# SKIRT/SKIRT9

Measured on AMD Instinct MI355X. Metric: photon packets/s (whole node), 10^6-cell octree, higher is better.
Workload: dtype f64

## Files before the change

### skirt9_amd/csrc/pmc_context.h

```cpp
#ifndef PMC_CONTEXT_H
#define PMC_CONTEXT_H

#include "pmc_device.h"
#include "../../include/pmc_layout.h"
#include "../../include/pmc_tuning.h"
#include <hip/hip_runtime.h>
#include <algorithm>
#include <chrono>
#include <cmath>
#include <cstdio>
#include <rccl/rccl.h>
#include <cstdlib>
#include <cstring>
#include <deque>
#include <atomic>
#include <mutex>
#include <string>
#include <thread>
#include <map>
#include <vector>

extern "C" const char* pmcTune(const char* name);
extern "C" hipError_t pmcUploadScene(int slot, const DevScene* scene, hipStream_t stream);
extern "C" hipError_t pmcConfigureKernels(size_t walkLds, size_t transitionLds);
extern "C" int pmcWalkBlocksPerCU(int gridKind, int kind, int wide, int block, size_t ldsBytes);
extern "C" hipError_t pmcLaunchStatMerge(int slot, int blocks, hipStream_t stream);
extern "C" int pmcPeelBlock(void);
extern "C" int pmcPropBlock(void);
extern "C" hipError_t pmcLaunchWalk(int slot, int gridKind, int flavour, int taskBase, int numTaskRecords, int taskCounter, uint64_t seed, int grid,
                                    int block, size_t ldsBytes, const WalkStreamArgs* tasks, hipStream_t stream);
extern "C" hipError_t pmcLaunchPeel(int slot, int form, int slotBase, int numSlots, const int* list, int cursor, int obs, int sgn, int grid, size_t ldsBytes,
                                    const PeelRec* sortedRec, const unsigned long long* sortedCount, unsigned long long* xcdCursor, hipStream_t stream);
extern "C" int pmcVoroPropWavesPerSimd(void);
extern "C" hipError_t pmcLaunchVoroProp(int slot, const int32_t* list, const unsigned long long* count, unsigned long long* xcdCursor, int segments, uint64_t seed,
                                        int flavour, int grid, hipStream_t stream);
extern "C" int pmcVoroPeelWavesPerSimd(void);
extern "C" hipError_t pmcLaunchVoroPeel(int slot, int rec, int tab, const int32_t* list, const unsigned long long* count, unsigned long long* xcdCursor, int segments,
                                        int severalMedia, int grid, hipStream_t stream);
extern "C" hipError_t pmcLaunchProp(int slot, int wide, int flavour, int checkpoints, int slotBase, int numSlots, const int* list, int cursor, uint64_t seed,
                                    int grid, size_t ldsBytes, const RfLogArgs* rfLog, hipStream_t stream);
extern "C" hipError_t pmcLaunchRfFlush(int slot, const uint32_t* keys, const double* vals, uint32_t* sortedKeys, double* sortedVals, unsigned long long n,
                                       int numParts, void* temp, int numCU, hipStream_t stream);
extern "C" int pmcPeelHasQueues(int form, size_t ldsBytes);
extern "C" int pmcPropHasCheckpoints(int flavour, size_t ldsBytes);
extern "C" int pmcExperimentBuild(void);
extern "C" const unsigned long long* pmcPeelSortedCount(void* temp);
extern "C" size_t pmcPeelSortTempBytes();
extern "C" hipError_t pmcLaunchPeelSortCounts(int slot, int slotBase, int numSlots, PeelSortArgs* ps, PeelRec* const* sorted, int32_t* const* lists, void* const* temp,
                                              int* groups, hipStream_t stream);
extern "C" size_t pmcRfTempBytes(int numParts);
extern "C" int pmcRfMaxParts();
extern "C" hipError_t pmcLaunchDipoleCosines(const double* u, int64_t n, double* out, hipStream_t stream);
extern "C" hipError_t pmcLaunchTransition(int slot, int dipole, int slotBase, int numSlots, int group, uint64_t seed, const int* list, int listLen, int maxBlocks,
                                          size_t ldsBytes, const StatLogArgs* statLog, uint64_t count, hipStream_t stream);
extern "C" hipError_t pmcLaunchLaunch(int slot, int slotBase, int numSlots, int group, uint64_t first, uint64_t count, uint64_t seed, int initial,
                                      int maxBlocks, size_t ldsBytes, const StatLogArgs* statLog, hipStream_t stream);
extern "C" hipError_t pmcLaunchStatFlush(int slot, const uint32_t* keys, const double* vals, uint32_t* sortedKeys, double* sortedVals, unsigned long long n,
                                         int numParts, void* temp, int numCU, const uint32_t* chunkFill, hipStream_t stream);
extern "C" int pmcStatBucketBits();
extern "C" hipError_t pmcLaunchCycleStart(int slot, int gridKind, int slotBase, int numSlots, int listCounter, int* listOut, const int* listIn,
                                          int listLen, int maxBlocks, size_t ldsBytes, const PeelSortArgs* sort, hipStream_t stream);
extern "C" hipError_t pmcLaunchTrace(int slot, int gridKind, int wide, int uniform, const double r[3], const double k[3],
                                     const double* kdev, int32_t* m, double* ds, int32_t cap, int32_t* n, size_t ldsBytes,
                                     hipStream_t stream);

void pmcSetError(const std::string& message);
namespace
{
    inline int fail(int code, const std::string& message)
    {
        pmcSetError(message);
        return code;
    }
    inline int hipFail(hipError_t e, const char* what)
    {
        return fail(PMC_ERR_DEVICE, std::string(what) + ": " + hipGetErrorString(e));
    }
}

#define HIP_TRY(call)                                           \
    do                                                          \
    {                                                           \
// ... 132 lines not shown
```

### skirt9_amd/csrc/pmc_device.h

```cpp
#ifndef PMC_DEVICE_H
#define PMC_DEVICE_H

#include "../../include/pmc.h"
#include <stdint.h>

#define PMC_MAX_INSTRUMENTS 16
#define PMC_MAX_CONTEXTS 6
#define PMC_MAX_LEVEL 20
#define PMC_STAT_CAP 48
#define PMC_STAT_POOL_EXHAUSTED 0x40000000

#define PMC_LINK_NONE 0x7FFFFFFFu
#define PMC_LINK_NODE 0x80000000u
#define PMC_LINK_OCTET 0x40000000u
#define PMC_LINK_EXP_BITS 5
#define PMC_LINK_EXP_MASK 31u
#define PMC_LINK_INDEX_MASK 0x1FFFFFFu
#define PMC_LINK_MAX_INDEX ((1u << 25) - 2u)

struct CellRec
{
    double   density;
    uint32_t link[6];
};
// ... 232 lines not shown
    int cursor;
    unsigned long long* waveBase;
    uint32_t* waveFill;
    uint32_t* chunkFill;
};
#define PMC_STAT_NO_CHUNK 0xFFFFFFFFu
#define PMC_STAT_LOG_WAVES 16384
#define PMC_STAT_BUCKET_BITS 11

struct PeelRec
{
    double rx, ry, rz;
    double ds;
    double target;
    uint64_t pidx;
    uint32_t cell, bits;
    int32_t slot;
    uint32_t pad;
};
#define PMC_SORT_OBS 4
struct PeelSortArgs
{
    int32_t numObs;
    int32_t propIndex;
    int32_t obs[PMC_SORT_OBS];
    int8_t sortIndex[16];
    PeelRec* out[PMC_SORT_OBS];
    int32_t* listOut[PMC_SORT_OBS];
    uint32_t* matrix[PMC_SORT_OBS];
    const unsigned long long* start[PMC_SORT_OBS];
    uint32_t numParts;
    uint32_t cap;
    int32_t ldsOffset;
    double centre[3];
    double scale;
};
struct WalkStreamArgs
{
    int32_t numLists;
    int32_t rec[PMC_SORT_OBS];
    const int32_t* list[PMC_SORT_OBS];
    const unsigned long long* count[PMC_SORT_OBS];
    unsigned long long* xcdCursor;
    const int32_t* propList;
    const unsigned long long* propCount;
};
struct PeelSortedArgs
{
    const PeelRec* rec;
    const unsigned long long* count;
    unsigned long long* xcdCursor;
};
#ifndef PMC_PEEL_TILES
#define PMC_PEEL_TILES 32
#endif
#define PMC_VORO_RUN_UNIT_BITS 27
#define PMC_VORO_RUN_UNIT_MASK 0x07FFFFFFu
#define PMC_VORO_RUN_COUNT_UNKNOWN 31u
#define PMC_VORO_FIRST_SCAN (-1000)
#define PMC_VORO_RUN_PAD 16
#ifndef PMC_VORO_RUN_LANES
#define PMC_VORO_RUN_LANES 2
#endif
#ifndef PMC_VORO_CONES
#define PMC_VORO_CONES 192
#endif
// ... 20 lines not shown
```

### skirt9_amd/csrc/pmc_kernels.hip

```cpp

#include "pmc_device.h"
#include "../../include/pmc_philox.h"
#include <hip/hip_runtime.h>
#include <cstdlib>
#include <cstring>
#include <float.h>
#include <math.h>
#include <algorithm>
#include <mutex>
#include <array>
#include <type_traits>
#include <utility>

#ifndef PMC_WALK_REFILL
    #define PMC_WALK_REFILL 40
#endif
#ifndef PMC_PEEL_REFILL
    #define PMC_PEEL_REFILL 32
#endif
#ifndef PMC_PROP_REFILL
    #define PMC_PROP_REFILL 40
#endif
#ifndef PMC_PEEL_BLOCK
    #define PMC_PEEL_BLOCK 768
// ... 314 lines not shown
{
    WalkStreamArgs ws;
    std::memset(&ws, 0, sizeof(ws));
    if (tasks) ws = *tasks;
    const WalkKernel kernel = walkKernels[(flavour & 7) | (gridKind == PMC_GRID_VORONOI ? 8 : 0)].kernel;
    hipLaunchKernelGGL(kernel, dim3(grid), dim3(block), ldsBytes, stream, slot, taskBase, numTaskRecords, taskCounter, seed, ws);
    return hipGetLastError();
}

extern "C" int pmcVoroPeelWavesPerSimd(void) { return PMC_VPEEL_MIN_WAVES; }
extern "C" hipError_t pmcLaunchVoroPeel(int slot, int rec, int tab, const int32_t* list, const unsigned long long* count, unsigned long long* xcdCursor, int segments,
                                        int severalMedia, int grid, hipStream_t stream)
{
    hipLaunchKernelGGL(severalMedia ? voroPeelKernel<true> : voroPeelKernel<false>, dim3(grid), dim3(256), 0, stream, slot, rec, tab, list, count, xcdCursor,
                       segments);
    return hipGetLastError();
}

extern "C" int pmcVoroPropWavesPerSimd(void) { return PMC_VPROP_MIN_WAVES; }
extern "C" hipError_t pmcLaunchVoroProp(int slot, const int32_t* list, const unsigned long long* count, unsigned long long* xcdCursor, int segments, uint64_t seed,
                                        int flavour, int grid, hipStream_t stream)
{
    hipLaunchKernelGGL(voroPropKernels[flavour & 7], dim3(grid), dim3(256), 0, stream, slot, list, count, xcdCursor, segments, seed);
    return hipGetLastError();
}

constexpr int PEEL_SORT_GROUPS = 1024;
constexpr int PEEL_SORT_PARTS = PMC_PEEL_TILES * PMC_PEEL_TILES;
extern "C" size_t pmcPeelSortTempBytes()
{
    return (size_t(2) * PEEL_SORT_PARTS + 2) * sizeof(unsigned long long) + size_t(PEEL_SORT_GROUPS) * PEEL_SORT_PARTS * sizeof(uint32_t);
}
extern "C" const unsigned long long* pmcPeelSortedCount(void* temp) { return static_cast<const unsigned long long*>(temp) + 2 * PEEL_SORT_PARTS; }
extern "C" hipError_t pmcLaunchPeelSortCounts(int slot, int slotBase, int numSlots, PeelSortArgs* ps, PeelRec* const* sorted, int32_t* const* lists, void* const* temp,
                                              int* groups, hipStream_t stream)
{
    ps->numParts = PEEL_SORT_PARTS;
    const int numLists = ps->numObs + (ps->propIndex >= 0 ? 1 : 0);
    for (int k = 0; k < numLists; ++k)
    {
        unsigned long long* totals = static_cast<unsigned long long*>(temp[k]);
        ps->out[k] = sorted ? sorted[k] : nullptr;
        ps->listOut[k] = lists ? lists[k] : nullptr;
        ps->matrix[k] = reinterpret_cast<uint32_t*>(totals + 2 * PEEL_SORT_PARTS + 2);
        ps->start[k] = totals + PEEL_SORT_PARTS;
    }
    const int tiles = (numSlots + PEEL_SORT_TILE - 1) / PEEL_SORT_TILE;
    *groups = std::max(1, std::min(tiles, PEEL_SORT_GROUPS));
    hipLaunchKernelGGL(peelSortCountKernel, dim3(*groups), dim3(256), 0, stream, slot, slotBase, numSlots, *ps);
    for (int k = 0; k < numLists; ++k)
    {
        unsigned long long* totals = static_cast<unsigned long long*>(temp[k]);
        hipLaunchKernelGGL(peelSortOffsetsKernel, dim3((PEEL_SORT_PARTS + 15) / 16), dim3(256), 0, stream, ps->matrix[k], (uint32_t)*groups, (uint32_t)PEEL_SORT_PARTS, totals);
        hipLaunchKernelGGL(rfScanKernel, dim3(1), dim3(PMC_SCAN_THREADS), 0, stream, totals, totals + PEEL_SORT_PARTS, (uint32_t)PEEL_SORT_PARTS);
    }
    return hipGetLastError();
}

extern "C" hipError_t pmcLaunchPeel(int slot, int form, int slotBase, int numSlots, const int* list, int cursor, int obs, int sgn, int grid, size_t ldsBytes,
                                    const PeelRec* sortedRec, const unsigned long long* sortedCount, unsigned long long* xcdCursor, hipStream_t stream)
{
    if (!(form & 4))
        hipLaunchKernelGGL(peelKernels[form & 3].kernel, dim3(grid), dim3(PMC_PEEL_BLOCK), ldsBytes, stream, slot, slotBase, numSlots, cursor, obs, list);
    else
    {
        const size_t queueOffset = (ldsBytes + 15) & ~size_t(15);
        const PeelSortedArgs sorted = {sortedRec, sortedCount, xcdCursor};
        hipLaunchKernelGGL(peel2Kernels[(form & 1) * 8 + (sgn & 7)].kernel, dim3(grid), dim3(PMC_PEEL_BLOCK), queueOffset + pmcPeelQueueBytes(), stream, slot,
                           slotBase, numSlots, cursor, obs, (int)queueOffset, list, sorted);
    }
    return hipGetLastError();
}

extern "C" hipError_t pmcLaunchProp(int slot, int wide, int flavour, int checkpoints, int slotBase, int numSlots, const int* list, int cursor, uint64_t seed,
                                    int grid, size_t ldsBytes, const RfLogArgs* rfLog, hipStream_t stream)
{
    const PropKernel kernel = propKernels[(flavour & 7) | (wide ? 8 : 0)].kernel;
    const size_t trimOffset = (ldsBytes + 15) & ~size_t(15);
    RfLogArgs none = {nullptr, nullptr, 0ull, 0, 0u};
    hipLaunchKernelGGL(kernel, dim3(grid), dim3(PMC_PROP_BLOCK), checkpoints ? trimOffset + PROP_CKPT_BYTES : ldsBytes, stream, slot, slotBase, numSlots, cursor,
                       seed, checkpoints ? (int)trimOffset : -1, rfLog ? *rfLog : none, list);
    return hipGetLastError();
// ... 122 lines not shown
```

### skirt9_amd/csrc/pmc_run.hip

```cpp
#include "pmc_context.h"

namespace
{
    int allocateSlotArrays(pmc_ctx* ctx, int64_t n);
    void releaseSlots(pmc_ctx* ctx)
    {
        for (void* p : ctx->slotAllocations) hipFree(p);
        ctx->slotAllocations.clear();
        ctx->allocatedSlots = 0;
    }

    int allocateSlots(pmc_ctx* ctx, int64_t n)
    {
        hipSetDevice(ctx->device);
        releaseSlots(ctx);
        ctx->planning = true;
        ctx->plannedBytes = 0;
        int rc = allocateSlotArrays(ctx, n);
        ctx->planning = false;
        if (rc) return rc;
        size_t freeBytes = 0, totalBytes = 0;
        if (!ctx->slotsConfigured && n > (int64_t(1) << 20) && hipMemGetInfo(&freeBytes, &totalBytes) == hipSuccess && ctx->plannedBytes > freeBytes / 2)
        {
            const int64_t less = std::max<int64_t>(int64_t(1) << 20, n / 2);
// ... 81 lines not shown
                if (hipMemcpy(ctx->statPoolIota, iota.data(), iota.size() * sizeof(int32_t), hipMemcpyHostToDevice) != hipSuccess)
                    return fail(PMC_ERR_DEVICE, "hipMemcpy failed");
                ctx->statPoolBlocks = blocks;
            }
        }
        TaskArrays& K = ctx->dev.tasks;
        std::memset(&K, 0, sizeof(K));
        const size_t nt = size_t(n) * size_t(1 + ctx->dev.num_instruments);
        double** tdbl[] = {&K.rx, &K.ry, &K.rz, &K.kx, &K.ky, &K.kz, &K.s0, &K.ds, &K.target};
        for (double** d : tdbl)
            if ((rc = ctx->allocate<double>(nt, d, false, &own))) return rc;
        int32_t** tints[] = {&K.cell, &K.cijk};
        for (int32_t** d : tints)
            if ((rc = ctx->allocate<int32_t>(nt, d, false, &own))) return rc;
        if ((rc = ctx->allocate<uint32_t>(size_t(n) / 64 + 64, &K.endedCount, true, &own))) return rc;
        if ((rc = ctx->allocate<int32_t>(2 * size_t(n), &K.liveList, false, &own))) return rc;
        if ((rc = ctx->allocate<uint32_t>(nt, &K.bits, false, &own))) return rc;
    if (ctx->dev.grid_kind == PMC_GRID_OCTREE && (rc = ctx->allocate<uint64_t>(nt, &K.pidx, false, &own))) return rc;
        if (ctx->planning) return PMC_OK;
        A.num_slots = n;
        ctx->allocatedSlots = n;
        ctx->sceneDirty = true;
        return PMC_OK;
    }
}

int pmcAllocateSlots(pmc_ctx* ctx, int64_t n)
{
    return allocateSlots(ctx, n);
}

namespace
{
    struct SegmentPlan
    {
        uint64_t first, count, seed;
        int G;
        int base[PMC_MAX_GROUPS], size[PMC_MAX_GROUPS];
        bool octree;
        int walkFlavour;
        int peelForm;
        bool propCheckpoints;
        int numSortObs, sortObs[PMC_SORT_OBS];
        int propSortIndex, numSortLists;
        PeelSortArgs sortArgs;
        bool sparseLists;
        int listTasksPerLane;
        bool rfLogged, statLogged;
        int rfBuckets, statParts;
        uint32_t rfPadKey;
        unsigned long long rfLogPerSlot, statLogEntries;
        bool poolGrows;
        int statInstruments;
        int launchBlocks, cycleBlocks, transitionBlocks;
        int voroPropGrid, voroPeelGrid, voroPropSegments;
        bool serialWalks, genDump, xcdAffinity, voroPeelKernels, voroPropKernel, voroWalksInSeries;
    };
    struct SegmentRun
    {
        bool active[PMC_MAX_GROUPS], haveWalk[PMC_MAX_GROUPS];
        bool listBuilt[PMC_MAX_GROUPS];
        int listHalf[PMC_MAX_GROUPS];
        bool peelSorted[PMC_MAX_GROUPS];
        bool poolCannotGrow;
        float walkMs, transMs, peelMs, propMs;
        int generations;
    };

    int provisionSlots(pmc_ctx* ctx, uint64_t count, int* numSlots)
    {
        const int64_t want = std::min<int64_t>(ctx->numSlots, (int64_t)std::min<uint64_t>(count, uint64_t(1) << 30));
        bool grow = want > ctx->allocatedSlots;
        if (grow && ctx->allocatedSlots > 0 && ctx->steppedDownFree)
        {
            size_t freeBytes = 0, totalBytes = 0;
            grow = hipMemGetInfo(&freeBytes, &totalBytes) == hipSuccess && freeBytes > ctx->steppedDownFree + ctx->steppedDownFree / 4;
        }
        if (grow)
        {
            HIP_TRY(hipStreamSynchronize(ctx->stream));
            ctx->steppedDownFree = 0;
            int rc = allocateSlots(ctx, want);
            if (rc) return rc;
        }
        *numSlots = (int)std::min<int64_t>(want, ctx->allocatedSlots);
        if (ctx->sceneDirty)
        {
            HIP_TRY(hipStreamSynchronize(ctx->stream));
            HIP_TRY(pmcUploadScene(ctx->slot, &ctx->dev, ctx->stream));
            ctx->sceneDirty = false;
        }
        return PMC_OK;
    }

    SegmentPlan planSegment(const pmc_ctx* ctx, int numSlots, uint64_t first, uint64_t count, uint64_t seed)
    {
        const DevScene& D = ctx->dev;
        SegmentPlan P;
        std::memset(&P, 0, sizeof(P));
        P.first = first, P.count = count, P.seed = seed;
        P.octree = D.grid_kind == PMC_GRID_OCTREE;
        P.serialWalks = pmcTune("PMC_SERIAL_WALKS") != nullptr;
        P.genDump = pmcTune("PMC_GEN_DUMP") != nullptr;
        const bool peelSort = pmcTune("PMC_NO_PEEL_SORT") == nullptr;
        int G = ctx->numGroups;
        if (numSlots < G * 65536) G = 1;
        {
            int observers = 0;
            for (int i = 0; i < D.num_instruments; ++i) observers += D.inst[i].same_observer ? 0 : 1;
            if (D.grid_kind == PMC_GRID_VORONOI && observers <= PMC_SORT_OBS && !ctx->groupsConfigured && peelSort) G = 1;
        }
        P.G = G;
        const int per = ((numSlots + G - 1) / G + PMC_TRANSITION_ALIGN - 1) / PMC_TRANSITION_ALIGN * PMC_TRANSITION_ALIGN;
        for (int g = 0; g < G; ++g)
        {
            P.base[g] = std::min(numSlots, g * per);
            P.size[g] = std::min(per, numSlots - P.base[g]);
        }
        P.walkFlavour = (D.rf_store ? 1 : 0) | (D.explicit_absorption ? 2 : 0) | (D.num_media > 1 ? 4 : 0);
        P.peelForm = (ctx->wide ? 1 : 0) | (D.num_media > 1 ? 2 : 0);
        if (pmcPeelHasQueues(P.peelForm, ctx->walkLds)) P.peelForm |= 4;
        P.propCheckpoints = pmcPropHasCheckpoints(P.walkFlavour, ctx->walkLds);
        P.propSortIndex = -1;
        if (peelSort && (!P.octree || (P.peelForm & 4)))
        {
            int observers = 0;
            for (int i = 0; i < D.num_instruments; ++i)
                if (!D.inst[i].same_observer)
                {
                    if (observers < PMC_SORT_OBS) P.sortObs[observers] = i;
                    ++observers;
                }
            if (observers <= PMC_SORT_OBS) P.numSortObs = observers;
        }
        if (!P.octree && P.numSortObs > 0 && P.numSortObs < PMC_SORT_OBS && pmcTune("PMC_NO_PROP_SORT") == nullptr) P.propSortIndex = P.numSortObs;
        P.numSortLists = P.numSortObs + (P.propSortIndex >= 0 ? 1 : 0);
        PeelSortArgs& sa = P.sortArgs;
        sa.numObs = P.numSortObs;
        sa.propIndex = P.propSortIndex;
        for (int i = 0; i < 16; ++i) sa.sortIndex[i] = -1;
        for (int k = 0; k < P.numSortObs; ++k) sa.obs[k] = P.sortObs[k], sa.sortIndex[P.sortObs[k]] = (int8_t)k;
        const double gdx = D.gx1 - D.gx0, gdy = D.gy1 - D.gy0, gdz = D.gz1 - D.gz0;
        sa.centre[0] = 0.5 * (D.gx0 + D.gx1), sa.centre[1] = 0.5 * (D.gy0 + D.gy1), sa.centre[2] = 0.5 * (D.gz0 + D.gz1);
        sa.scale = PMC_PEEL_TILES / std::sqrt(gdx * gdx + gdy * gdy + gdz * gdz);
        P.xcdAffinity = pmcTune("PMC_NO_XCD_AFFINITY") == nullptr;
        P.sparseLists = P.octree && pmcTune("PMC_NO_LIVE_LISTS") == nullptr;
        P.listTasksPerLane = 1;
        if (const char* env = pmcTune("PMC_LIST_TASKS_PER_LANE")) P.listTasksPerLane = std::max(1, atoi(env));
        P.voroPeelKernels = D.grid_kind == PMC_GRID_VORONOI && pmcTune("PMC_VORO_NO_PEEL_KERNEL") == nullptr;
        P.voroPropKernel = D.grid_kind == PMC_GRID_VORONOI && D.vgen_run && pmcTune("PMC_VORO_NO_PROP_KERNEL") == nullptr
                           && !(pmcTune("PMC_VORO_PLAIN_PROP_ONLY") && (D.num_media > 1 || D.rf_store || D.explicit_absorption));
        P.voroWalksInSeries = pmcTune("PMC_VORO_WALKS_IN_SERIES") != nullptr;
        P.voroPropSegments = (P.xcdAffinity && pmcTune("PMC_VPROP_XCD_SEGMENTS")) ? 8 : 1;
        int propBlocks = pmcVoroPropWavesPerSimd(), peelBlocks = pmcVoroPeelWavesPerSimd();
        if (const char* v = pmcTune("PMC_VPROP_BLOCKS_PER_CU")) propBlocks = std::max(1, atoi(v));
        if (const char* v = pmcTune("PMC_VPEEL_BLOCKS_PER_CU")) peelBlocks = std::max(1, atoi(v));
        P.voroPropGrid = ctx->numCU * propBlocks, P.voroPeelGrid = ctx->numCU * peelBlocks;
        const int64_t rfKeys = P.octree ? int64_t(D.cell_slots) * D.rf_num_lambda : ctx->rfSize;
        const int64_t rfParts = (rfKeys + (int64_t(1) << PMC_RF_BUCKET_BITS) - 1) >> PMC_RF_BUCKET_BITS;
        P.rfLogged = D.rf_store && P.octree && rfParts <= pmcRfMaxParts() && pmcTune("PMC_RF_ATOMICS") == nullptr;
        if (D.rf_store && P.octree && rfParts > pmcRfMaxParts())
        {
            static std::atomic<bool> said{false};
            if (!said.exchange(true))
                fprintf(stderr, "libpmc: the radiation field table has %lld entries, more than the log's counting sort partitions (%d x %d): contributions are added atomically\n",
                        (long long)rfKeys, pmcRfMaxParts(), 1 << PMC_RF_BUCKET_BITS);
        }
        P.rfBuckets = P.rfLogged ? int(rfParts) : 0;
        P.rfPadKey = uint32_t(P.rfBuckets) << PMC_RF_BUCKET_BITS;
        P.rfLogPerSlot = 128ull;
        if (const char* env = pmcTune("PMC_RF_LOG_PER_SLOT")) P.rfLogPerSlot = std::max(1, atoi(env));
        const int statBits = pmcStatBucketBits();
        P.statParts = int((D.stat_acc_records + (int64_t(1) << statBits) - 1) >> statBits);
        P.statLogged = D.any_stats && D.stat_acc_records > 0 && P.statParts <= pmcRfMaxParts() && pmcTune("PMC_STAT_ATOMICS") == nullptr;
        unsigned long long entries = (128ull << 20);
        if (const char* env = pmcTune("PMC_STAT_LOG_ENTRIES")) entries = std::max(1, atoi(env));
        P.statLogEntries = std::max<unsigned long long>((entries + PMC_RF_LOG_CHUNK - 1) / PMC_RF_LOG_CHUNK, 1ull) * PMC_RF_LOG_CHUNK;
        for (int i = 0; i < D.num_instruments; ++i) P.statInstruments += D.inst[i].record_stats ? 1 : 0;
        P.poolGrows = D.any_stats && ctx->statPoolBlocks > 0 && pmcTune("PMC_STAT_POOL_NO_GROWTH") == nullptr;
// ... 219 lines not shown
            D.stat_pool_first[h] = first;
            D.stat_pool_count[h] = count;
            first += count;
        }
        freeNow[g] += (unsigned long long)add;
        HIP_TRY(hipMemcpy(ctr + PMC_CTR_STATFREE(0), freeNow, sizeof(freeNow), hipMemcpyHostToDevice));
        ctx->release(D.stat_pool_bin, own), ctx->release(D.stat_pool_w, own), ctx->release(D.stat_pool_next, own), ctx->release(D.stat_pool_free, own);
        ctx->release(ctx->statPoolIota, own);
        D.stat_pool_bin = bin, D.stat_pool_w = w, D.stat_pool_next = next, D.stat_pool_free = stack;
        ctx->statPoolIota = iota;
        ctx->statPoolBlocks = old + add;
        ctx->readback[g].statFreeBlocks = freeNow[g];
        ctx->statPoolGrowths += 1;
        HIP_TRY(pmcUploadScene(ctx->slot, &D, ctx->stream));
        HIP_TRY(hipStreamSynchronize(ctx->stream));
        return PMC_OK;
    }

    int enqueueOctreeWalks(pmc_ctx* ctx, const SegmentPlan& P, const SegmentRun& S, int g, const int* listIn, int listLen)
    {
        const DevScene& D = ctx->dev;
        hipStream_t sg = ctx->groupStream[g], sp = P.serialWalks ? sg : ctx->peelStream[g];
        const int numTasks = listIn ? listLen : P.size[g];
        const int peelLanes = pmcPeelBlock() * P.listTasksPerLane, propLanes = pmcPropBlock() * P.listTasksPerLane;
        const int peelGrid = listIn ? std::max(1, std::min(ctx->peelGrid, (numTasks + peelLanes - 1) / peelLanes)) : ctx->peelGrid;
        const int propGrid = listIn ? std::max(1, std::min(ctx->grid, (numTasks + propLanes - 1) / propLanes)) : ctx->grid;
        HIP_TRY(hipStreamWaitEvent(sp, ctx->evA[g], 0));
        for (int i = 0; i < D.num_instruments; ++i)
            if (!D.inst[i].same_observer)
            {
                int k = -1;
                for (int q = 0; q < P.numSortObs; ++q)
                    if (P.sortObs[q] == i) k = q;
                const bool sorted = S.peelSorted[g] && !listIn && k >= 0;
                HIP_TRY(pmcLaunchPeel(ctx->slot, P.peelForm, P.base[g], numTasks, sorted ? nullptr : listIn, PMC_CTR_TASK(g, 1 + i), i, (int)D.inst[i].sgn, peelGrid,
                                      ctx->walkLds, sorted ? ctx->peelRec[g][k] : nullptr, sorted ? pmcPeelSortedCount(ctx->peelTemp[g][k]) : nullptr,
                                      sorted && P.xcdAffinity ? cursorSet(ctx, g, k) : nullptr, sp));
            }
        HIP_TRY(hipEventRecord(ctx->evJoin[g], sp));
        RfLogArgs log = {ctx->rfKeys[g][0], ctx->rfVals[g][0], P.rfLogged ? ctx->rfCap[g] : 0ull, PMC_CTR_RFLOG(g), P.rfPadKey};
        if (P.serialWalks) HIP_TRY(hipEventRecord(ctx->evProp[g], sg));
        HIP_TRY(pmcLaunchProp(ctx->slot, ctx->wide, P.walkFlavour, P.propCheckpoints, P.base[g], numTasks, listIn, PMC_CTR_TASK(g, 0), P.seed, propGrid, ctx->walkLds,
                              &log, sg));
        if (!P.serialWalks) HIP_TRY(hipEventRecord(ctx->evProp[g], sg));
        HIP_TRY(hipStreamWaitEvent(sg, ctx->evJoin[g], 0));
        return PMC_OK;
    }

    int enqueueGenericWalks(pmc_ctx* ctx, const SegmentPlan& P, const SegmentRun& S, int g)
    {
        const DevScene& D = ctx->dev;
        hipStream_t sg = ctx->groupStream[g];
        auto ownPeel = [&](int k) { return P.voroPeelKernels && D.vobs_of_inst[P.sortObs[k]] >= 0; };
        WalkStreamArgs tasks;
        std::memset(&tasks, 0, sizeof(tasks));
        bool streamEmpty = false;
        if (S.peelSorted[g])
        {
            tasks.numLists = P.numSortObs;
            for (int k = 0; k < P.numSortObs; ++k)
                tasks.rec[k] = 1 + P.sortObs[k], tasks.list[k] = ctx->peelList[g][k], tasks.count[k] = pmcPeelSortedCount(ctx->peelTemp[g][k]);
            tasks.xcdCursor = P.xcdAffinity ? cursorSet(ctx, g, 0) : nullptr;
            if (P.propSortIndex >= 0)
                tasks.propList = ctx->peelList[g][P.propSortIndex], tasks.propCount = pmcPeelSortedCount(ctx->peelTemp[g][P.propSortIndex]);
            bool left = false;
            for (int k = 0; k < P.numSortObs; ++k)
                if (ownPeel(k))
// ... 7 lines not shown
                tasks.propCount = zeroCount(ctx);
            }
            else
                left = true;
            streamEmpty = !left;
        }
        if (!streamEmpty)
            HIP_TRY(pmcLaunchWalk(ctx->slot, D.grid_kind, P.walkFlavour, P.base[g], P.size[g], PMC_CTR_TASK(g, 0), P.seed, ctx->grid, ctx->block, ctx->walkLds,
                                  S.peelSorted[g] ? &tasks : nullptr, sg));
        if (!S.peelSorted[g]) return PMC_OK;
        bool anyPeel = false;
        for (int k = 0; k < P.numSortObs; ++k) anyPeel = anyPeel || ownPeel(k);
        const bool side = anyPeel && P.voroPropKernel && P.propSortIndex >= 0 && !P.serialWalks && !P.voroWalksInSeries;
        hipStream_t sp = side ? ctx->peelStream[g] : sg;
        if (side) HIP_TRY(hipStreamWaitEvent(sp, ctx->evA[g], 0));
        for (int k = 0; k < P.numSortObs; ++k)
            if (ownPeel(k))
                HIP_TRY(pmcLaunchVoroPeel(ctx->slot, 1 + P.sortObs[k], D.vobs_of_inst[P.sortObs[k]], ctx->peelList[g][k], pmcPeelSortedCount(ctx->peelTemp[g][k]),
                                          cursorSet(ctx, g, 1 + k), P.xcdAffinity ? 8 : 1, D.num_media > 1 ? 1 : 0, P.voroPeelGrid, sp));
        if (side)
        {
            HIP_TRY(hipEventRecord(ctx->evJoin[g], sp));
            HIP_TRY(hipStreamWaitEvent(sg, ctx->evJoin[g], 0));
        }
        return PMC_OK;
    }

    int enqueueCycleStart(pmc_ctx* ctx, const SegmentPlan& P, SegmentRun& S, int g, bool initial, const int* listIn, int listLen)
    {
        DevScene& D = ctx->dev;
        hipStream_t sg = ctx->groupStream[g];
        unsigned long long* ctr = D.counters;
        GroupReadback& rb = ctx->readback[g];
        const bool buildList = P.sparseLists && !initial && (listIn || rb.live < (unsigned long long)(P.size[g] / 2));
        if (listIn) S.listHalf[g] ^= 1;
        int* const listOut = D.tasks.liveList + int64_t(S.listHalf[g]) * D.slots.num_slots + P.base[g];
        const bool sortNow = P.numSortObs > 0 && !buildList && !listIn;
        PeelSortArgs sortArgs = P.sortArgs;
        sortArgs.cap = (uint32_t)ctx->peelCap[g];
        int sortGroups = 0;
        if (sortNow)
            HIP_TRY(pmcLaunchPeelSortCounts(ctx->slot, P.base[g], P.size[g], &sortArgs, P.octree ? ctx->peelRec[g] : nullptr, P.octree ? nullptr : ctx->peelList[g],
                                            ctx->peelTemp[g], &sortGroups, sg));
        HIP_TRY(pmcLaunchCycleStart(ctx->slot, D.grid_kind, P.base[g], P.size[g], buildList ? PMC_CTR_LIST(g) : -1, listOut, listIn, listLen,
                                    sortNow ? sortGroups : P.cycleBlocks, ctx->walkLds, sortNow ? &sortArgs : nullptr, sg));
        S.peelSorted[g] = sortNow;
        S.listBuilt[g] = buildList;
        HIP_TRY(hipEventRecord(ctx->evC[g], sg));
        const size_t word = sizeof(unsigned long long);
        HIP_TRY(hipMemcpyAsync(&rb.live, ctr + PMC_CTR_LIVE(g), word, hipMemcpyDeviceToHost, sg));
        if (P.rfLogged && !initial) HIP_TRY(hipMemcpyAsync(&rb.rfLogFill, ctr + PMC_CTR_RFLOG(g), word, hipMemcpyDeviceToHost, sg));
        if (ctx->progress) HIP_TRY(hipMemcpyAsync(&rb.historyCursor, ctr + PMC_CTR_HISTORY, word, hipMemcpyDeviceToHost, sg));
        if (P.statLogged && !initial && ctx->statCap[g]) HIP_TRY(hipMemcpyAsync(&rb.statLogFill, ctr + PMC_CTR_STATLOG(g), word, hipMemcpyDeviceToHost, sg));
        if (P.poolGrows) HIP_TRY(hipMemcpyAsync(&rb.statFreeBlocks, ctr + PMC_CTR_STATFREE(g), word, hipMemcpyDeviceToHost, sg));
        return PMC_OK;
    }

    int enqueueGeneration(pmc_ctx* ctx, const SegmentPlan& P, SegmentRun& S, int g, bool initial)
    {
        const DevScene& D = ctx->dev;
        hipStream_t sg = ctx->groupStream[g];
        unsigned long long* ctr = D.counters;
        GroupReadback& rb = ctx->readback[g];
        int* const listIn = (!initial && S.listBuilt[g]) ? D.tasks.liveList + int64_t(S.listHalf[g]) * D.slots.num_slots + P.base[g] : nullptr;
        const int listLen = listIn ? int(rb.live) : 0;
        if (initial)
        {
            if (g > 0) HIP_TRY(hipStreamWaitEvent(sg, ctx->evStart, 0));
            HIP_TRY(hipEventRecord(ctx->evB[g], sg));
            HIP_TRY(pmcLaunchLaunch(ctx->slot, P.base[g], P.size[g], g, P.first, P.count, P.seed, 1, (P.size[g] + 255) / 256, ctx->launchLds, nullptr, sg));
            return enqueueCycleStart(ctx, P, S, g, initial, listIn, listLen);
        }
        if (P.poolGrows)
        {
            const int64_t need = int64_t(rb.live) * P.statInstruments, freeBlocks = int64_t(rb.statFreeBlocks);
            const bool inUse = freeBlocks < int64_t(D.stat_pool_count[g]) || D.min_scatt_events > 16;
// ... 53 lines not shown
                if (P.octree)
                {
                    HIP_TRY(hipEventElapsedTime(&ms, ctx->evA[g], ctx->evJoin[g]));
                    S.peelMs += ms;
                    if (P.serialWalks)
                        HIP_TRY(hipEventElapsedTime(&ms, ctx->evProp[g], ctx->evB[g]));
                    else
                        HIP_TRY(hipEventElapsedTime(&ms, ctx->evA[g], ctx->evProp[g]));
                    S.propMs += ms;
                }
            }
            HIP_TRY(hipEventElapsedTime(&ms, ctx->evB[g], ctx->evC[g]));
            S.transMs += ms;
            if (rb.live == 0)
            {
                if (int rc = rfFlush(ctx, P, g, rb.rfLogFill)) return rc;
                rb.rfLogFill = 0;
                S.active[g] = false;
                --remaining;
                continue;
            }
            ++S.generations;
            if (ctx->progress)
            {
                const auto now = std::chrono::steady_clock::now();
                if (std::chrono::duration<double>(now - lastReport).count() >= ctx->progressInterval)
                {
                    lastReport = now;
                    reported = std::max<uint64_t>(reported, std::min<uint64_t>(rb.historyCursor, P.count));
                    ctx->progress(ctx->progressUser, reported, P.count);
                }
            }
            if (P.genDump)
                fprintf(stderr, "PMC_GEN %d group %d live %llu walk_ms %.3f transition_ms %.3f at_ms %.3f\n", S.generations, g, rb.live,
                        S.haveWalk[g] ? walkOfGen : 0.f, ms, 1e3 * std::chrono::duration<double>(std::chrono::steady_clock::now() - segmentStart).count());
            if (int rc = enqueueGeneration(ctx, P, S, g, false)) return rc;
        }
        return PMC_OK;
    }

    int finish(pmc_ctx* ctx, const SegmentPlan& P)
    {
        if (P.statLogged)
            for (int g = 0; g < P.G; ++g)
                if (int rc = statFlush(ctx, P, g, ctx->readback[g].statLogFill, ctx->groupStream[g])) return rc;
        if (P.rfLogged || P.statLogged)
            for (int g = 0; g < P.G; ++g) HIP_TRY(hipStreamSynchronize(ctx->groupStream[g]));
        if (ctx->dev.stat_acc_records) HIP_TRY(pmcLaunchStatMerge(ctx->slot, ctx->numCU * 8, ctx->stream));
        HIP_TRY(hipEventRecord(ctx->evStop, ctx->stream));
        HIP_TRY(hipEventSynchronize(ctx->evStop));
        HIP_TRY(hipEventElapsedTime(&ctx->totalMs, ctx->evStart, ctx->evStop));
        return PMC_OK;
    }

    int abandon(pmc_ctx* ctx, int code)
    {
        hipDeviceSynchronize();
        if (ctx->dev.stat_acc_records) hipMemset(ctx->dev.stat_acc, 0, size_t(ctx->dev.stat_acc_records) * 8 * sizeof(double));
        ctx->timed = false;
        return code;
    }

    int checkKernelErrors(pmc_ctx* ctx)
    {
        const unsigned long long* ctr = ctx->dev.counters;
        {
            unsigned long long tail[3] = {0, 0, 0};
            HIP_TRY(hipMemcpy(tail, ctr + 5, sizeof(tail), hipMemcpyDeviceToHost));
// ... 54 lines not shown
```

### skirt9_amd/csrc/pmc_transition.inc

```

    struct DustLds
    {
        const double* lamb;
        const double* sext;
        const double* ssca;
        const double* asym;
        const double* src;
        double* sed;
        unsigned long long* hotKey;
        double* hotVal;
    };
    constexpr int HOT_BINS = 256;

    struct PhaseHG
    {
        double g;
        double onePlusG2;
        double twoG;
        double norm;
        __device__ __forceinline__ explicit PhaseHG(double asym) : g(asym), onePlusG2(1. + asym * asym), twoG(2. * asym), norm((1. - asym) * (1. + asym)) {}
        __device__ __forceinline__ double kernel(double c) const { return onePlusG2 - twoG * c; }
        __device__ __forceinline__ double value(double c) const
        {
            const double t = kernel(c);
// ... 1528 lines not shown
                    }
                    assigned = false;
                    if (event == EV_LAUNCH)
                    {
                        if (h >= bound)
                        {
                            event = EV_DEAD;
                            A.mode[slot] = MODE_NONE;
                            for (int r = 0; r <= S.num_instruments; ++r) S.tasks.bits[(int64_t)r * A.num_slots + slot] = PMC_TASK_NONE;
                        }
                        else
                        {
                            cnt.histories += 1;
                            if (launchHistory(S, L, cnt, slot, first + h, seed)) event = EV_TASK;
                        }
                    }
                }
                if (event == EV_TASK) liveCount += 1;
                PMC_T_STAMP(3);
            }
            __builtin_amdgcn_wave_barrier();
        }
        {
            const unsigned long long live = waveSum(liveCount);
            if (lane == 0 && live) atomicAdd(S.counters + PMC_CTR_LIVE(group), live);
        }
        statLogEnd(statLog, logWave, lane);
        flushBlock(S, L, tid, blockDim.x);
        PMC_T_STAMP(6);
        PMC_T_PROF_END(200);
        addCounters(S, cnt, lane);
    }

    template<int GRID>
    __global__ __launch_bounds__(256, PMC_CYCLE_MIN_WAVES) void cycleStartKernel(const int sceneSlot, const int slotBase, const int numSlots,
                                                                                 const int listCounter, int* const listOut,
                                                                                 const int* const listIn, const int listLen, const PeelSortArgs ps)
    {
        const DevScene& S = c_scene[sceneSlot];
        extern __shared__ double lds[];
        const int tid = threadIdx.x;
        const int lane = tid & 63;
        if (GRID == GRID_TREE) requireLdsBaseZero(lds);
        stageGrid<GRID>(S, lds, tid, blockDim.x);
        __syncthreads();
        const GridLds G = makeGridLds(S, lds);
        const SlotArrays& A = S.slots;
        Counters cnt = {0, 0, 0, 0, 0};
        const int slotEnd = slotBase + numSlots;
        const bool sparse = GRID == GRID_TREE && listIn != nullptr;
        if (ps.numObs > 0 && !sparse)
        {
            uint32_t* const cur = reinterpret_cast<uint32_t*>(reinterpret_cast<char*>(lds) + ps.ldsOffset);
            const int numLists = ps.numObs + (ps.propIndex >= 0 ? 1 : 0);
            for (int k = 0; k < numLists; ++k)
                for (uint32_t p = tid; p < ps.numParts; p += blockDim.x)
                    cur[(uint32_t)k * ps.numParts + p] = (uint32_t)ps.start[k][p] + ps.matrix[k][(size_t)blockIdx.x * ps.numParts + p];
            __syncthreads();
            const int tiles = (numSlots + PEEL_SORT_TILE - 1) / PEEL_SORT_TILE;
            for (int t = blockIdx.x; t < tiles; t += gridDim.x)
                for (int i = t * PEEL_SORT_TILE + tid; i < (t + 1) * PEEL_SORT_TILE && i < numSlots; i += blockDim.x)
                {
                    const int slot = slotBase + i;
                    const int md = A.mode[slot];
                    if (md & MODE_ALIVE) startCycleWalks<GRID>(S, G, cnt, slot, md, &ps, cur);
                }
        }
        else
        {
            const int end = sparse ? listLen : numSlots;
            for (int i0 = blockIdx.x * blockDim.x; i0 < end; i0 += gridDim.x * blockDim.x)
            {
                const int i = i0 + tid;
                const int slot = sparse ? (i < listLen ? listIn[i] : -1) : slotBase + i;
                const int md = (slot >= 0 && slot < slotEnd) ? A.mode[slot] : 0;
                if (md & MODE_ALIVE) startCycleWalks<GRID>(S, G, cnt, slot, md);
                if (GRID == GRID_TREE && listCounter >= 0)
                {
                    const unsigned long long m = __ballot((md & MODE_ALIVE) != 0);
                    if (m)
                    {
                        unsigned long long at = 0;
                        if (lane == __ffsll((long long)m) - 1) at = atomicAdd(S.counters + listCounter, (unsigned long long)__popcll(m));
                        at = __shfl(at, __ffsll((long long)m) - 1, 64);
                        if (md & MODE_ALIVE) listOut[(int)at + __popcll(m & ((1ull << lane) - 1ull))] = slot;
                    }
                }
            }
        }
        const unsigned long long v = waveSum(cnt.paths);
        if (lane == 0 && v) atomicAdd(S.counters + 1, v);
    }

    __global__ __launch_bounds__(256) void peelSortCountKernel(const int sceneSlot, const int slotBase, const int numSlots, const PeelSortArgs ps)
    {
        const DevScene& S = c_scene[sceneSlot];
        const SlotArrays& A = S.slots;
        __shared__ uint32_t h[PMC_SORT_OBS * PMC_PEEL_TILES * PMC_PEEL_TILES];
        const int tid = threadIdx.x;
        const int numLists = ps.numObs + (ps.propIndex >= 0 ? 1 : 0);
        for (uint32_t p = tid; p < (uint32_t)numLists * ps.numParts; p += blockDim.x) h[p] = 0u;
        __syncthreads();
        const int tiles = (numSlots + PEEL_SORT_TILE - 1) / PEEL_SORT_TILE;
        for (int t = blockIdx.x; t < tiles; t += gridDim.x)
            for (int i = t * PEEL_SORT_TILE + tid; i < (t + 1) * PEEL_SORT_TILE && i < numSlots; i += blockDim.x)
            {
                const int slot = slotBase + i;
                const int md = A.mode[slot];
                if (!(md & MODE_ALIVE)) continue;
                const double x = A.rx[slot], y = A.ry[slot], z = A.rz[slot];
                for (int k = 0; k < ps.numObs; ++k)
                    if (((uint32_t)md >> (8 + ps.obs[k])) & 1u) atomicAdd(&h[(uint32_t)k * ps.numParts + peelTile(ps, S.inst[ps.obs[k]], x, y, z)], 1u);
                if (ps.propIndex >= 0)
                    atomicAdd(&h[(uint32_t)ps.propIndex * ps.numParts + propSortKey(S, x, y, z, A.kx[slot], A.ky[slot], A.kz[slot])], 1u);
            }
        __syncthreads();
        for (int k = 0; k < numLists; ++k)
            for (uint32_t p = tid; p < ps.numParts; p += blockDim.x) ps.matrix[k][(size_t)blockIdx.x * ps.numParts + p] = h[(uint32_t)k * ps.numParts + p];
    }
    __global__ __launch_bounds__(256) void peelSortOffsetsKernel(uint32_t* __restrict__ matrix, const uint32_t groups, const uint32_t numParts,
                                                                 unsigned long long* __restrict__ totals)
    {
        __shared__ uint32_t part[16][17];
        const uint32_t pl = threadIdx.x & 15u, run = threadIdx.x >> 4;
        const uint32_t p = blockIdx.x * 16u + pl;
        const uint32_t rows = (groups + 15u) / 16u;
        const uint32_t b0 = run * rows, b1 = b0 + rows < groups ? b0 + rows : groups;
        uint32_t sum = 0u;
        if (p < numParts)
            for (uint32_t b = b0; b < b1; ++b) sum += matrix[(size_t)b * numParts + p];
        part[run][pl] = sum;
        __syncthreads();
        uint32_t before = 0u, all = 0u;
        for (uint32_t r = 0; r < 16u; ++r)
        {
            const uint32_t v = part[r][pl];
            if (r < run) before += v;
            all += v;
        }
        if (p < numParts)
// ... 11 lines not shown
```

Before: 206.6 million.

## Enable peel sorting over sparse live lists and tune list-build threshold

Extends the peel-sort count and cycle-start kernels so they can iterate over a compacted live-slot list instead of only over the full slot range. Sorted peel-off can now also be used in generations that run from sparse lists, as long as the live count exceeds a minimum, with an adaptive tile size. The list-build threshold and the group-split minimum become tunable. The aim is to keep the coherence benefit of sorted peel records in late generations, at the cost of an extra sort-count pass over those lists.

```diff
diff --git a/skirt9_amd/csrc/pmc_context.h b/skirt9_amd/csrc/pmc_context.h
--- a/skirt9_amd/csrc/pmc_context.h
+++ b/skirt9_amd/csrc/pmc_context.h
@@ -46,8 +46,8 @@
 extern "C" int pmcExperimentBuild(void);
 extern "C" const unsigned long long* pmcPeelSortedCount(void* temp);
 extern "C" size_t pmcPeelSortTempBytes();
-extern "C" hipError_t pmcLaunchPeelSortCounts(int slot, int slotBase, int numSlots, PeelSortArgs* ps, PeelRec* const* sorted, int32_t* const* lists, void* const* temp,
-                                              int* groups, hipStream_t stream);
+extern "C" hipError_t pmcLaunchPeelSortCounts(int slot, int slotBase, int numSlots, const int* list, int listLen, PeelSortArgs* ps, PeelRec* const* sorted,
+                                              int32_t* const* lists, void* const* temp, int* groups, hipStream_t stream);
 extern "C" size_t pmcRfTempBytes(int numParts);
 extern "C" int pmcRfMaxParts();
 extern "C" hipError_t pmcLaunchDipoleCosines(const double* u, int64_t n, double* out, hipStream_t stream);
diff --git a/skirt9_amd/csrc/pmc_device.h b/skirt9_amd/csrc/pmc_device.h
--- a/skirt9_amd/csrc/pmc_device.h
+++ b/skirt9_amd/csrc/pmc_device.h
@@ -288,6 +288,7 @@
     uint32_t numParts;
     uint32_t cap;
     int32_t ldsOffset;
+    int32_t tile;
     double centre[3];
     double scale;
 };
diff --git a/skirt9_amd/csrc/pmc_kernels.hip b/skirt9_amd/csrc/pmc_kernels.hip
--- a/skirt9_amd/csrc/pmc_kernels.hip
+++ b/skirt9_amd/csrc/pmc_kernels.hip
@@ -370,10 +370,12 @@
     return (size_t(2) * PEEL_SORT_PARTS + 2) * sizeof(unsigned long long) + size_t(PEEL_SORT_GROUPS) * PEEL_SORT_PARTS * sizeof(uint32_t);
 }
 extern "C" const unsigned long long* pmcPeelSortedCount(void* temp) { return static_cast<const unsigned long long*>(temp) + 2 * PEEL_SORT_PARTS; }
-extern "C" hipError_t pmcLaunchPeelSortCounts(int slot, int slotBase, int numSlots, PeelSortArgs* ps, PeelRec* const* sorted, int32_t* const* lists, void* const* temp,
-                                              int* groups, hipStream_t stream)
+extern "C" hipError_t pmcLaunchPeelSortCounts(int slot, int slotBase, int numSlots, const int* list, int listLen, PeelSortArgs* ps, PeelRec* const* sorted,
+                                              int32_t* const* lists, void* const* temp, int* groups, hipStream_t stream)
 {
     ps->numParts = PEEL_SORT_PARTS;
+    const int entries = list ? listLen : numSlots;
+    ps->tile = list ? std::min(PEEL_SORT_TILE, std::max(256, (entries / PEEL_SORT_GROUPS + 255) / 256 * 256)) : PEEL_SORT_TILE;
     const int numLists = ps->numObs + (ps->propIndex >= 0 ? 1 : 0);
     for (int k = 0; k < numLists; ++k)
     {
@@ -383,9 +385,9 @@
         ps->matrix[k] = reinterpret_cast<uint32_t*>(totals + 2 * PEEL_SORT_PARTS + 2);
         ps->start[k] = totals + PEEL_SORT_PARTS;
     }
-    const int tiles = (numSlots + PEEL_SORT_TILE - 1) / PEEL_SORT_TILE;
+    const int tiles = (entries + ps->tile - 1) / ps->tile;
     *groups = std::max(1, std::min(tiles, PEEL_SORT_GROUPS));
-    hipLaunchKernelGGL(peelSortCountKernel, dim3(*groups), dim3(256), 0, stream, slot, slotBase, numSlots, *ps);
+    hipLaunchKernelGGL(peelSortCountKernel, dim3(*groups), dim3(256), 0, stream, slot, slotBase, numSlots, list, listLen, *ps);
     for (int k = 0; k < numLists; ++k)
     {
         unsigned long long* totals = static_cast<unsigned long long*>(temp[k]);
diff --git a/skirt9_amd/csrc/pmc_run.hip b/skirt9_amd/csrc/pmc_run.hip
--- a/skirt9_amd/csrc/pmc_run.hip
+++ b/skirt9_amd/csrc/pmc_run.hip
@@ -137,6 +137,8 @@
 
 namespace
 {
+    constexpr int PMC_LIST_BELOW_PERCENT = 50;
+    constexpr int PMC_LIST_SORT_MIN = 16384;
     struct SegmentPlan
     {
         uint64_t first, count, seed;
@@ -150,6 +152,9 @@
         int propSortIndex, numSortLists;
         PeelSortArgs sortArgs;
         bool sparseLists;
+        int listBelowPercent;
+        bool listSort;
+        int listSortMin;
         int listTasksPerLane;
         bool rfLogged, statLogged;
         int rfBuckets, statParts;
@@ -209,7 +214,9 @@
         P.genDump = pmcTune("PMC_GEN_DUMP") != nullptr;
         const bool peelSort = pmcTune("PMC_NO_PEEL_SORT") == nullptr;
         int G = ctx->numGroups;
-        if (numSlots < G * 65536) G = 1;
+        int minGroupSlots = 65536;
+        if (const char* v = pmcTune("PMC_MIN_GROUP_SLOTS")) minGroupSlots = std::max(1, atoi(v));
+        if (numSlots < int64_t(G) * minGroupSlots) G = 1;
         {
             int observers = 0;
             for (int i = 0; i < D.num_instruments; ++i) observers += D.inst[i].same_observer ? 0 : 1;
@@ -250,6 +257,11 @@
         sa.scale = PMC_PEEL_TILES / std::sqrt(gdx * gdx + gdy * gdy + gdz * gdz);
         P.xcdAffinity = pmcTune("PMC_NO_XCD_AFFINITY") == nullptr;
         P.sparseLists = P.octree && pmcTune("PMC_NO_LIVE_LISTS") == nullptr;
+        P.listBelowPercent = PMC_LIST_BELOW_PERCENT;
+        if (const char* v = pmcTune("PMC_LIST_BELOW_PERCENT")) P.listBelowPercent = std::max(0, std::min(100, atoi(v)));
+        P.listSort = pmcTune("PMC_NO_LIST_SORT") == nullptr;
+        P.listSortMin = PMC_LIST_SORT_MIN;
+        if (const char* v = pmcTune("PMC_LIST_SORT_MIN")) P.listSortMin = std::max(0, atoi(v));
         P.listTasksPerLane = 1;
         if (const char* env = pmcTune("PMC_LIST_TASKS_PER_LANE")) P.listTasksPerLane = std::max(1, atoi(env));
         P.voroPeelKernels = D.grid_kind == PMC_GRID_VORONOI && pmcTune("PMC_VORO_NO_PEEL_KERNEL") == nullptr;
@@ -535,7 +547,7 @@
                 int k = -1;
                 for (int q = 0; q < P.numSortObs; ++q)
                     if (P.sortObs[q] == i) k = q;
-                const bool sorted = S.peelSorted[g] && !listIn && k >= 0;
+                const bool sorted = S.peelSorted[g] && k >= 0;
                 HIP_TRY(pmcLaunchPeel(ctx->slot, P.peelForm, P.base[g], numTasks, sorted ? nullptr : listIn, PMC_CTR_TASK(g, 1 + i), i, (int)D.inst[i].sgn, peelGrid,
                                       ctx->walkLds, sorted ? ctx->peelRec[g][k] : nullptr, sorted ? pmcPeelSortedCount(ctx->peelTemp[g][k]) : nullptr,
                                       sorted && P.xcdAffinity ? cursorSet(ctx, g, k) : nullptr, sp));
@@ -609,16 +621,16 @@
         hipStream_t sg = ctx->groupStream[g];
         unsigned long long* ctr = D.counters;
         GroupReadback& rb = ctx->readback[g];
-        const bool buildList = P.sparseLists && !initial && (listIn || rb.live < (unsigned long long)(P.size[g] / 2));
+        const bool buildList = P.sparseLists && !initial && (listIn || rb.live * 100ull < (unsigned long long)P.size[g] * (unsigned long long)P.listBelowPercent);
         if (listIn) S.listHalf[g] ^= 1;
         int* const listOut = D.tasks.liveList + int64_t(S.listHalf[g]) * D.slots.num_slots + P.base[g];
-        const bool sortNow = P.numSortObs > 0 && !buildList && !listIn;
+        const bool sortNow = P.numSortObs > 0 && ((!buildList && !listIn) || (P.listSort && rb.live >= (unsigned long long)P.listSortMin));
         PeelSortArgs sortArgs = P.sortArgs;
         sortArgs.cap = (uint32_t)ctx->peelCap[g];
         int sortGroups = 0;
         if (sortNow)
-            HIP_TRY(pmcLaunchPeelSortCounts(ctx->slot, P.base[g], P.size[g], &sortArgs, P.octree ? ctx->peelRec[g] : nullptr, P.octree ? nullptr : ctx->peelList[g],
-                                            ctx->peelTemp[g], &sortGroups, sg));
+            HIP_TRY(pmcLaunchPeelSortCounts(ctx->slot, P.base[g], P.size[g], listIn, listLen, &sortArgs, P.octree ? ctx->peelRec[g] : nullptr,
+                                            P.octree ? nullptr : ctx->peelList[g], ctx->peelTemp[g], &sortGroups, sg));
         HIP_TRY(pmcLaunchCycleStart(ctx->slot, D.grid_kind, P.base[g], P.size[g], buildList ? PMC_CTR_LIST(g) : -1, listOut, listIn, listLen,
                                     sortNow ? sortGroups : P.cycleBlocks, ctx->walkLds, sortNow ? &sortArgs : nullptr, sg));
         S.peelSorted[g] = sortNow;
@@ -738,8 +750,9 @@
                 }
             }
             if (P.genDump)
-                fprintf(stderr, "PMC_GEN %d group %d live %llu walk_ms %.3f transition_ms %.3f at_ms %.3f\n", S.generations, g, rb.live,
-                        S.haveWalk[g] ? walkOfGen : 0.f, ms, 1e3 * std::chrono::duration<double>(std::chrono::steady_clock::now() - segmentStart).count());
+                fprintf(stderr, "PMC_GEN %d group %d live %llu walk_ms %.3f transition_ms %.3f at_ms %.3f form %s%s\n", S.generations, g, rb.live,
+                        S.haveWalk[g] ? walkOfGen : 0.f, ms, 1e3 * std::chrono::duration<double>(std::chrono::steady_clock::now() - segmentStart).count(),
+                        S.listBuilt[g] ? "list" : "slots", S.peelSorted[g] ? "+sorted" : "");
             if (int rc = enqueueGeneration(ctx, P, S, g, false)) return rc;
         }
         return PMC_OK;
diff --git a/skirt9_amd/csrc/pmc_transition.inc b/skirt9_amd/csrc/pmc_transition.inc
--- a/skirt9_amd/csrc/pmc_transition.inc
+++ b/skirt9_amd/csrc/pmc_transition.inc
@@ -1584,6 +1584,15 @@
         addCounters(S, cnt, lane);
     }
 
+    __device__ __forceinline__ void appendLiveSlot(const DevScene& S, int listCounter, int* listOut, int slot, bool alive, int lane)
+    {
+        const unsigned long long m = __ballot(alive);
+        if (!m) return;
+        unsigned long long at = 0;
+        if (lane == __ffsll((long long)m) - 1) at = atomicAdd(S.counters + listCounter, (unsigned long long)__popcll(m));
+        at = __shfl(at, __ffsll((long long)m) - 1, 64);
+        if (alive) listOut[(int)at + __popcll(m & ((1ull << lane) - 1ull))] = slot;
+    }
     template<int GRID>
     __global__ __launch_bounds__(256, PMC_CYCLE_MIN_WAVES) void cycleStartKernel(const int sceneSlot, const int slotBase, const int numSlots,
                                                                                  const int listCounter, int* const listOut,
@@ -1601,7 +1610,8 @@
         Counters cnt = {0, 0, 0, 0, 0};
         const int slotEnd = slotBase + numSlots;
         const bool sparse = GRID == GRID_TREE && listIn != nullptr;
-        if (ps.numObs > 0 && !sparse)
+        const int end = sparse ? listLen : numSlots;
+        if (ps.numObs > 0)
         {
             uint32_t* const cur = reinterpret_cast<uint32_t*>(reinterpret_cast<char*>(lds) + ps.ldsOffset);
             const int numLists = ps.numObs + (ps.propIndex >= 0 ? 1 : 0);
@@ -1609,42 +1619,37 @@
                 for (uint32_t p = tid; p < ps.numParts; p += blockDim.x)
                     cur[(uint32_t)k * ps.numParts + p] = (uint32_t)ps.start[k][p] + ps.matrix[k][(size_t)blockIdx.x * ps.numParts + p];
             __syncthreads();
-            const int tiles = (numSlots + PEEL_SORT_TILE - 1) / PEEL_SORT_TILE;
+            const int tiles = (end + ps.tile - 1) / ps.tile;
             for (int t = blockIdx.x; t < tiles; t += gridDim.x)
-                for (int i = t * PEEL_SORT_TILE + tid; i < (t + 1) * PEEL_SORT_TILE && i < numSlots; i += blockDim.x)
-                {
-                    const int slot = slotBase + i;
-                    const int md = A.mode[slot];
+            {
+                const int tileEnd = min((t + 1) * ps.tile, end);
+                for (int i0 = t * ps.tile; i0 < tileEnd; i0 += blockDim.x)
+                {
+                    const int i = i0 + tid;
+                    const int slot = i < tileEnd ? (sparse ? listIn[i] : slotBase + i) : -1;
+                    const int md = (slot >= 0 && slot < slotEnd) ? A.mode[slot] : 0;
                     if (md & MODE_ALIVE) startCycleWalks<GRID>(S, G, cnt, slot, md, &ps, cur);
-                }
+                    if (GRID == GRID_TREE && listCounter >= 0) appendLiveSlot(S, listCounter, listOut, slot, (md & MODE_ALIVE) != 0, lane);
+                }
+            }
         }
         else
         {
-            const int end = sparse ? listLen : numSlots;
             for (int i0 = blockIdx.x * blockDim.x; i0 < end; i0 += gridDim.x * blockDim.x)
             {
                 const int i = i0 + tid;
                 const int slot = sparse ? (i < listLen ? listIn[i] : -1) : slotBase + i;
                 const int md = (slot >= 0 && slot < slotEnd) ? A.mode[slot] : 0;
                 if (md & MODE_ALIVE) startCycleWalks<GRID>(S, G, cnt, slot, md);
-                if (GRID == GRID_TREE && listCounter >= 0)
-                {
-                    const unsigned long long m = __ballot((md & MODE_ALIVE) != 0);
-                    if (m)
-                    {
-                        unsigned long long at = 0;
-                        if (lane == __ffsll((long long)m) - 1) at = atomicAdd(S.counters + listCounter, (unsigned long long)__popcll(m));
-                        at = __shfl(at, __ffsll((long long)m) - 1, 64);
-                        if (md & MODE_ALIVE) listOut[(int)at + __popcll(m & ((1ull << lane) - 1ull))] = slot;
-                    }
-                }
+                if (GRID == GRID_TREE && listCounter >= 0) appendLiveSlot(S, listCounter, listOut, slot, (md & MODE_ALIVE) != 0, lane);
             }
         }
         const unsigned long long v = waveSum(cnt.paths);
         if (lane == 0 && v) atomicAdd(S.counters + 1, v);
     }
 
-    __global__ __launch_bounds__(256) void peelSortCountKernel(const int sceneSlot, const int slotBase, const int numSlots, const PeelSortArgs ps)
+    __global__ __launch_bounds__(256) void peelSortCountKernel(const int sceneSlot, const int slotBase, const int numSlots, const int* const list, const int listLen,
+                                                               const PeelSortArgs ps)
     {
         const DevScene& S = c_scene[sceneSlot];
         const SlotArrays& A = S.slots;
@@ -1653,11 +1658,13 @@
         const int numLists = ps.numObs + (ps.propIndex >= 0 ? 1 : 0);
         for (uint32_t p = tid; p < (uint32_t)numLists * ps.numParts; p += blockDim.x) h[p] = 0u;
         __syncthreads();
-        const int tiles = (numSlots + PEEL_SORT_TILE - 1) / PEEL_SORT_TILE;
+        const int end = list ? listLen : numSlots;
+        const int tiles = (end + ps.tile - 1) / ps.tile;
         for (int t = blockIdx.x; t < tiles; t += gridDim.x)
-            for (int i = t * PEEL_SORT_TILE + tid; i < (t + 1) * PEEL_SORT_TILE && i < numSlots; i += blockDim.x)
-            {
-                const int slot = slotBase + i;
+            for (int i = t * ps.tile + tid; i < (t + 1) * ps.tile && i < end; i += blockDim.x)
+            {
+                const int slot = list ? list[i] : slotBase + i;
+                if (slot < 0 || slot >= slotBase + numSlots) continue;
                 const int md = A.mode[slot];
                 if (!(md & MODE_ALIVE)) continue;
                 const double x = A.rx[slot], y = A.ry[slot], z = A.rz[slot];
```

New measurement: 206.1 million. About the same (-0.2%).
